# ElementsProject/lightning

Hardware: NVIDIA H100
Metric: secp256k1 verifies/sec (higher is better)
Workload: dtype u32 (8x32-bit limbs, IMAD.WIDE.U32 carry chains)

## Files before the change

### include/cln_sigverify.h

```cpp
#ifndef CLN_SIGVERIFY_H
#define CLN_SIGVERIFY_H

#include <stddef.h>
#include <stdint.h>

#ifdef __cplusplus
extern "C" {
#endif

typedef struct sv_ctx sv_ctx;

#define SV_KIND_ECDSA33 0
#define SV_KIND_ECDSA_XY 1
#define SV_KIND_SCHNORR 2

typedef enum {
    SV_OK = 0,
    SV_ERR_NO_DEVICE = -1,
    SV_ERR_CUDA = -2,
    SV_ERR_NOMEM = -3,
    SV_ERR_ARG = -4
} sv_status;

int sv_create(sv_ctx **out, int device);
// ... 63 lines not shown
int sv_pubkey_parse_host(sv_ctx *ctx, const uint8_t *key33, size_t n, uint8_t *xy64, uint8_t *ok);

enum {
    SV_ST_FE_MUL = 0,
    SV_ST_FE_SQR = 1,
    SV_ST_FE_ADD = 2,
    SV_ST_FE_SUB = 3,
    SV_ST_FE_NEG = 4,
    SV_ST_FE_NORMALIZE = 5,
    SV_ST_FE_INV = 6,
    SV_ST_FE_SQRT = 7,
    SV_ST_FE_MUL3 = 8,
    SV_ST_FE_MUL8 = 9,
    SV_ST_FE_MUL_SMALL = 10,
    SV_ST_FE_DBL = 11,
    SV_ST_FE_B32 = 12,
    SV_ST_U256_MUL_WIDE = 13,
    SV_ST_U256_SQR_WIDE = 14,
    SV_ST_FE_REDUCE512 = 15,
    SV_ST_U256_ADD = 16,
    SV_ST_U256_SUB = 17,
    SV_ST_SC_MUL = 20,
    SV_ST_SC_SQR = 21,
    SV_ST_SC_ADD = 22,
    SV_ST_SC_NEGATE = 23,
    SV_ST_SC_INVERSE = 24,
    SV_ST_SC_REDUCE512 = 25,
    SV_ST_SC_SPLIT_LAMBDA = 26,
    SV_ST_SC_SET_B32 = 27,
    SV_ST_ECMULT_GEN = 28,
    SV_ST_PREPARE_U2 = 29,
    SV_ST_PREPARE_U1 = 30,
    SV_ST_SC_INVERSE_VAR = 31,
    SV_ST_FE_INV_VAR = 32
};
int sv_selftest_host(sv_ctx *ctx, int op, const uint32_t *a, const uint32_t *b, size_t n, uint32_t *out);

int sv_synth_device(sv_ctx *ctx, int kind, uint64_t seed, size_t n, void *d_msg32, void *d_key, void *d_sig64,
                    void *stream);

typedef struct {
    int device;
    int sm_count;
    int main_block;
    int main_grid;
    int main_regs;
    size_t gtable_bytes;
    size_t scratch_bytes;
    unsigned long long launches;
    size_t l2_persist_bytes;
    size_t l2_max_persist_bytes;
} sv_info;
int sv_get_info(const sv_ctx *ctx, sv_info *info);

int sv_set_profiling(sv_ctx *ctx, int on);
int sv_get_last_timing(sv_ctx *ctx, float *prep_ms, float *main_ms);

int sv_probe_imad_peak(sv_ctx *ctx, double *imad_per_sec);
int sv_probe(sv_ctx *ctx, int mode, double *ops_per_sec);

void *sv_host_alloc(size_t bytes);
void sv_host_free(void *p);

#ifdef __cplusplus
}
#endif
#endif
// ... 1 lines not shown
```

### lightning_b200/csrc/engine.cu

```cuda
#include <cuda_runtime.h>
#include <stdio.h>
#include <stdlib.h>
#include <string.h>
#include <string>
#include <vector>

#include "../../include/cln_sigverify.h"
#include "verify.cuh"
#include "selftest.cuh"
#include "batch.cuh"

#if !defined(SV_NO_SYNC_INLINE) && !defined(SV_FE_INLINE)
#error "compile with -DSV_FE_INLINE -DSV_MAIN_SYNC (default build) or -DSV_NO_SYNC_INLINE; see lightning_b200/build.py"
#endif
#ifndef SV_MAIN_BLOCK
#ifdef SV_MAIN_SYNC
#define SV_MAIN_BLOCK 256
#else
#define SV_MAIN_BLOCK 128
#endif
#endif
#ifndef SV_MAIN_MINB
#define SV_MAIN_MINB (512 / SV_MAIN_BLOCK)
#endif
// ... 1676 lines not shown
    memcpy(it.sig, sig64, 64);
    ctx->queue.push_back(it);
    return (long)ctx->queue.size() - 1;
}
extern "C" size_t sv_pending(const sv_ctx* ctx) { return ctx ? ctx->queue.size() : 0; }

extern "C" int sv_flush(sv_ctx* ctx, uint8_t* verdicts, size_t capacity) {
    if (!ctx || (!verdicts && !ctx->queue.empty())) return SV_ERR_ARG;
    size_t total = ctx->queue.size();
    if (capacity < total) return SV_ERR_ARG;
    for (int kind = 0; kind < 3; kind++) {
        size_t ks = sv_key_size(kind);
        std::vector<size_t> idx;
        for (size_t i = 0; i < total; i++)
            if (ctx->queue[i].kind == kind) idx.push_back(i);
        if (idx.empty()) continue;
        size_t m = idx.size();
        std::vector<u8> msg(32 * m), key(ks * m), sig(64 * m), out(m);
        for (size_t j = 0; j < m; j++) {
            const sv_queue_item& it = ctx->queue[idx[j]];
            memcpy(&msg[32 * j], it.msg, 32);
            memcpy(&key[ks * j], it.key, ks);
            memcpy(&sig[64 * j], it.sig, 64);
        }
        int rc = sv_verify_host(ctx, kind, msg.data(), key.data(), sig.data(), m, out.data());
        if (rc) return rc;
        for (size_t j = 0; j < m; j++) verdicts[idx[j]] = out[j];
    }
    ctx->queue.clear();
    return SV_OK;
}

extern "C" int sv_selftest_host(sv_ctx* ctx, int op, const uint32_t* a, const uint32_t* b, size_t n, uint32_t* out) {
    if (!ctx || op < 0 || op > SV_ST_FE_INV_VAR || (n && (!a || !b || !out))) return SV_ERR_ARG;
    if (n == 0) return SV_OK;
    dev_guard dg__;
    CK(dg__.enter(ctx->device));
    dev_tmp ta, tb, to;
    CK(ta.alloc(n * 32));
    CK(tb.alloc(n * 32));
    CK(to.alloc(n * 64));
    cudaStream_t st = ctx->stream;
    CK(cudaMemcpyAsync(ta.p, a, n * 32, cudaMemcpyHostToDevice, st));
    CK(cudaMemcpyAsync(tb.p, b, n * 32, cudaMemcpyHostToDevice, st));
    k_selftest<<<(unsigned)((n + 127) / 128), 128, 0, st>>>(op, ta.as<u32>(), tb.as<u32>(), n, to.as<u32>(), ctx->d_gtab);
    ctx->launches += 1;
    CK(cudaGetLastError());
    CK(cudaMemcpyAsync(out, to.p, n * 64, cudaMemcpyDeviceToHost, st));
    CK(cudaStreamSynchronize(st));
    return SV_OK;
}

extern "C" int sv_synth_device(sv_ctx* ctx, int kind, uint64_t seed, size_t n, void* d_msg32, void* d_key,
                               void* d_sig64, void* stream) {
    if (!ctx || sv_key_size(kind) == 0 || (n && (!d_msg32 || !d_key || !d_sig64))) return SV_ERR_ARG;
    if (n == 0) return SV_OK;
    dev_guard dg__;
    CK(dg__.enter(ctx->device));
    cudaStream_t st = stream ? (cudaStream_t)stream : ctx->stream;
    unsigned grid = (unsigned)((n + 127) / 128);
    if (kind == SV_KIND_ECDSA33)
        k_synth<SV_KIND_ECDSA33><<<grid, 128, 0, st>>>(seed, n, ctx->d_gtab, (u8*)d_msg32, (u8*)d_key, (u8*)d_sig64);
    else if (kind == SV_KIND_ECDSA_XY)
        k_synth<SV_KIND_ECDSA_XY><<<grid, 128, 0, st>>>(seed, n, ctx->d_gtab, (u8*)d_msg32, (u8*)d_key, (u8*)d_sig64);
    else
        k_synth<SV_KIND_SCHNORR><<<grid, 128, 0, st>>>(seed, n, ctx->d_gtab, (u8*)d_msg32, (u8*)d_key, (u8*)d_sig64);
    ctx->launches += 1;
// ... 53 lines not shown
```

### lightning_b200/csrc/fe.cuh

```cuda
#pragma once
#include "u256.cuh"

struct fe {
    u32 v[8];
};

#define SV_P0 0xFFFFFC2Fu
#define SV_P1 0xFFFFFFFEu
#define SV_PC 977u

SV_HD void fe_set_zero(fe& r) {
    SV_UNROLL
    for (int i = 0; i < 8; i++) r.v[i] = 0;
}
SV_HD void fe_set_u32(fe& r, u32 x) {
    fe_set_zero(r);
    r.v[0] = x;
}

SV_HD bool fe_gte_p(const fe& a) {
    u32 hi = a.v[7] & a.v[6] & a.v[5] & a.v[4] & a.v[3] & a.v[2];
    return (hi == 0xFFFFFFFFu) && ((a.v[1] == 0xFFFFFFFFu) || (a.v[1] == SV_P1 && a.v[0] >= SV_P0));
}

// ... 103 lines not shown
            "subc.cc.u32 %5, %5, 0;\n\t"
            "subc.u32 %6, 0, 0;"
            : "+r"(r.v[2]), "+r"(r.v[3]), "+r"(r.v[4]), "+r"(r.v[5]), "+r"(r.v[6]), "+r"(r.v[7]), "=r"(b2));
        b2 &= 1u;
        u32 k2 = b2 * SV_PC;
        asm("sub.cc.u32 %0, %0, %3;\n\t"
            "subc.u32 %1, %1, %2;"
            : "+r"(r.v[0]), "+r"(r.v[1])
            : "r"(b2), "r"(k2));
    }
#else
    u64 d = (u64)r.v[0] - (u64)bw * SV_PC;
    r.v[0] = (u32)d;
    u64 br = (d >> 32) & 1;
    d = (u64)r.v[1] - bw - br;
    r.v[1] = (u32)d;
    br = (d >> 32) & 1;
    for (int i = 2; i < 8; i++) { d = (u64)r.v[i] - br; r.v[i] = (u32)d; br = (d >> 32) & 1; }
    u32 b2 = (u32)br;
    d = (u64)r.v[0] - (u64)b2 * SV_PC;
    r.v[0] = (u32)d;
    br = (d >> 32) & 1;
    r.v[1] = (u32)((u64)r.v[1] - b2 - br);
#endif
}

SV_HD void fe_neg(fe& r, const fe& a) {
    fe z;
    fe_set_zero(z);
    fe_sub(r, z, a);
}
SV_HD void fe_dbl(fe& r, const fe& a) { fe_add(r, a, a); }

SV_HD void fe_reduce512(fe& r, const u32 t[16]) {
#if SV_DEVICE_CODE && defined(SV_REDUCE_SHIFTS)
    u32 s[10];
    s[0] = t[0];
    asm("add.cc.u32 %0, %9, %17;\n\t"
        "addc.cc.u32 %1, %10, %18;\n\t"
        "addc.cc.u32 %2, %11, %19;\n\t"
        "addc.cc.u32 %3, %12, %20;\n\t"
        "addc.cc.u32 %4, %13, %21;\n\t"
        "addc.cc.u32 %5, %14, %22;\n\t"
        "addc.cc.u32 %6, %15, %23;\n\t"
        "addc.cc.u32 %7, %16, 0;\n\t"
        "addc.u32 %8, 0, 0;"
        : "=r"(s[1]), "=r"(s[2]), "=r"(s[3]), "=r"(s[4]), "=r"(s[5]), "=r"(s[6]), "=r"(s[7]), "=r"(s[8]), "=r"(s[9])
        : "r"(t[8]), "r"(t[9]), "r"(t[10]), "r"(t[11]), "r"(t[12]), "r"(t[13]), "r"(t[14]), "r"(t[15]),
          "r"(t[1]), "r"(t[2]), "r"(t[3]), "r"(t[4]), "r"(t[5]), "r"(t[6]), "r"(t[7]));
    u32 h4[9];
    h4[0] = t[8] << 4;
    SV_UNROLL
    for (int k = 1; k < 8; k++) h4[k] = __funnelshift_l(t[8 + k - 1], t[8 + k], 4);
    h4[8] = t[15] >> 28;
    u32 a17[9], a15[9];
    asm("add.cc.u32 %0, %9, %18;\n\t"
        "addc.cc.u32 %1, %10, %19;\n\t"
        "addc.cc.u32 %2, %11, %20;\n\t"
        "addc.cc.u32 %3, %12, %21;\n\t"
        "addc.cc.u32 %4, %13, %22;\n\t"
        "addc.cc.u32 %5, %14, %23;\n\t"
        "addc.cc.u32 %6, %15, %24;\n\t"
        "addc.cc.u32 %7, %16, %25;\n\t"
        "addc.u32 %8, %17, 0;"
        : "=r"(a17[0]), "=r"(a17[1]), "=r"(a17[2]), "=r"(a17[3]), "=r"(a17[4]), "=r"(a17[5]), "=r"(a17[6]), "=r"(a17[7]), "=r"(a17[8])
        : "r"(h4[0]), "r"(h4[1]), "r"(h4[2]), "r"(h4[3]), "r"(h4[4]), "r"(h4[5]), "r"(h4[6]), "r"(h4[7]), "r"(h4[8]),
          "r"(t[8]), "r"(t[9]), "r"(t[10]), "r"(t[11]), "r"(t[12]), "r"(t[13]), "r"(t[14]), "r"(t[15]));
    asm("sub.cc.u32 %0, %9, %18;\n\t"
        "subc.cc.u32 %1, %10, %19;\n\t"
        "subc.cc.u32 %2, %11, %20;\n\t"
        "subc.cc.u32 %3, %12, %21;\n\t"
        "subc.cc.u32 %4, %13, %22;\n\t"
        "subc.cc.u32 %5, %14, %23;\n\t"
        "subc.cc.u32 %6, %15, %24;\n\t"
        "subc.cc.u32 %7, %16, %25;\n\t"
        "subc.u32 %8, %17, 0;"
        : "=r"(a15[0]), "=r"(a15[1]), "=r"(a15[2]), "=r"(a15[3]), "=r"(a15[4]), "=r"(a15[5]), "=r"(a15[6]), "=r"(a15[7]), "=r"(a15[8])
        : "r"(h4[0]), "r"(h4[1]), "r"(h4[2]), "r"(h4[3]), "r"(h4[4]), "r"(h4[5]), "r"(h4[6]), "r"(h4[7]), "r"(h4[8]),
          "r"(t[8]), "r"(t[9]), "r"(t[10]), "r"(t[11]), "r"(t[12]), "r"(t[13]), "r"(t[14]), "r"(t[15]));
    u32 b[9];
    b[0] = a15[0] << 6;
    SV_UNROLL
    for (int k = 1; k < 9; k++) b[k] = __funnelshift_l(a15[k - 1], a15[k], 6);
    asm("add.cc.u32 %0, %0, %10;\n\t"
        "addc.cc.u32 %1, %1, %11;\n\t"
        "addc.cc.u32 %2, %2, %12;\n\t"
        "addc.cc.u32 %3, %3, %13;\n\t"
        "addc.cc.u32 %4, %4, %14;\n\t"
        "addc.cc.u32 %5, %5, %15;\n\t"
        "addc.cc.u32 %6, %6, %16;\n\t"
        "addc.cc.u32 %7, %7, %17;\n\t"
        "addc.cc.u32 %8, %8, %18;\n\t"
        "addc.u32 %9, %9, 0;"
        : "+r"(s[0]), "+r"(s[1]), "+r"(s[2]), "+r"(s[3]), "+r"(s[4]), "+r"(s[5]), "+r"(s[6]), "+r"(s[7]), "+r"(s[8]), "+r"(s[9])
        : "r"(a17[0]), "r"(a17[1]), "r"(a17[2]), "r"(a17[3]), "r"(a17[4]), "r"(a17[5]), "r"(a17[6]), "r"(a17[7]), "r"(a17[8]));
    asm("add.cc.u32 %0, %0, %10;\n\t"
        "addc.cc.u32 %1, %1, %11;\n\t"
        "addc.cc.u32 %2, %2, %12;\n\t"
        "addc.cc.u32 %3, %3, %13;\n\t"
        "addc.cc.u32 %4, %4, %14;\n\t"
        "addc.cc.u32 %5, %5, %15;\n\t"
        "addc.cc.u32 %6, %6, %16;\n\t"
        "addc.cc.u32 %7, %7, %17;\n\t"
        "addc.cc.u32 %8, %8, %18;\n\t"
        "addc.u32 %9, %9, 0;"
        : "+r"(s[0]), "+r"(s[1]), "+r"(s[2]), "+r"(s[3]), "+r"(s[4]), "+r"(s[5]), "+r"(s[6]), "+r"(s[7]), "+r"(s[8]), "+r"(s[9])
        : "r"(b[0]), "r"(b[1]), "r"(b[2]), "r"(b[3]), "r"(b[4]), "r"(b[5]), "r"(b[6]), "r"(b[7]), "r"(b[8]));
    u64 T = ((u64)s[9] << 32) | s[8];
    u64 m = T * SV_PC;
    u64 mid = (m >> 32) + T;
    u32 f0 = (u32)m, f1 = (u32)mid, f2 = (u32)(mid >> 32);
    u32 c;
    asm("add.cc.u32 %0, %9, %17;\n\t"
        "addc.cc.u32 %1, %10, %18;\n\t"
        "addc.cc.u32 %2, %11, %19;\n\t"
        "addc.cc.u32 %3, %12, 0;\n\t"
        "addc.cc.u32 %4, %13, 0;\n\t"
        "addc.cc.u32 %5, %14, 0;\n\t"
        "addc.cc.u32 %6, %15, 0;\n\t"
        "addc.cc.u32 %7, %16, 0;\n\t"
        "addc.u32 %8, 0, 0;"
        : "=r"(r.v[0]), "=r"(r.v[1]), "=r"(r.v[2]), "=r"(r.v[3]), "=r"(r.v[4]), "=r"(r.v[5]), "=r"(r.v[6]),
          "=r"(r.v[7]), "=r"(c)
        : "r"(s[0]), "r"(s[1]), "r"(s[2]), "r"(s[3]), "r"(s[4]), "r"(s[5]), "r"(s[6]), "r"(s[7]), "r"(f0), "r"(f1),
          "r"(f2));
    asm("mad.lo.cc.u32 %0, %3, 977, %0;\n\t"
        "addc.cc.u32 %1, %1, %3;\n\t"
        "addc.u32 %2, %2, 0;"
        : "+r"(r.v[0]), "+r"(r.v[1]), "+r"(r.v[2])
        : "r"(c));
#elif SV_DEVICE_CODE
    u32 s[10];
    s[0] = t[0];
    asm("add.cc.u32 %0, %9, %17;\n\t"
        "addc.cc.u32 %1, %10, %18;\n\t"
        "addc.cc.u32 %2, %11, %19;\n\t"
        "addc.cc.u32 %3, %12, %20;\n\t"
        "addc.cc.u32 %4, %13, %21;\n\t"
        "addc.cc.u32 %5, %14, %22;\n\t"
        "addc.cc.u32 %6, %15, %23;\n\t"
        "addc.cc.u32 %7, %16, 0;\n\t"
        "addc.u32 %8, 0, 0;"
        : "=r"(s[1]), "=r"(s[2]), "=r"(s[3]), "=r"(s[4]), "=r"(s[5]), "=r"(s[6]), "=r"(s[7]), "=r"(s[8]), "=r"(s[9])
        : "r"(t[8]), "r"(t[9]), "r"(t[10]), "r"(t[11]), "r"(t[12]), "r"(t[13]), "r"(t[14]), "r"(t[15]),
          "r"(t[1]), "r"(t[2]), "r"(t[3]), "r"(t[4]), "r"(t[5]), "r"(t[6]), "r"(t[7]));
#ifdef SV_REDUCE_NOACC
    u32 pe[8];
    asm("mul.lo.u32 %0, %8, %12;\n\t"
        "mul.hi.u32 %1, %8, %12;\n\t"
        "mul.lo.u32 %2, %9, %12;\n\t"
        "mul.hi.u32 %3, %9, %12;\n\t"
        "mul.lo.u32 %4, %10, %12;\n\t"
        "mul.hi.u32 %5, %10, %12;\n\t"
        "mul.lo.u32 %6, %11, %12;\n\t"
        "mul.hi.u32 %7, %11, %12;"
        : "=r"(pe[0]), "=r"(pe[1]), "=r"(pe[2]), "=r"(pe[3]), "=r"(pe[4]), "=r"(pe[5]), "=r"(pe[6]), "=r"(pe[7])
        : "r"(t[8]), "r"(t[10]), "r"(t[12]), "r"(t[14]), "r"(SV_PC));
    asm("add.cc.u32 %0, %0, %10;\n\t"
        "addc.cc.u32 %1, %1, %11;\n\t"
        "addc.cc.u32 %2, %2, %12;\n\t"
        "addc.cc.u32 %3, %3, %13;\n\t"
        "addc.cc.u32 %4, %4, %14;\n\t"
        "addc.cc.u32 %5, %5, %15;\n\t"
        "addc.cc.u32 %6, %6, %16;\n\t"
        "addc.cc.u32 %7, %7, %17;\n\t"
        "addc.cc.u32 %8, %8, 0;\n\t"
        "addc.u32 %9, %9, 0;"
        : "+r"(s[0]), "+r"(s[1]), "+r"(s[2]), "+r"(s[3]), "+r"(s[4]), "+r"(s[5]), "+r"(s[6]), "+r"(s[7]),
          "+r"(s[8]), "+r"(s[9])
        : "r"(pe[0]), "r"(pe[1]), "r"(pe[2]), "r"(pe[3]), "r"(pe[4]), "r"(pe[5]), "r"(pe[6]), "r"(pe[7]));
#else
    asm("mad.lo.cc.u32 %0, %10, %14, %0;\n\t"
        "madc.hi.cc.u32 %1, %10, %14, %1;\n\t"
        "madc.lo.cc.u32 %2, %11, %14, %2;\n\t"
        "madc.hi.cc.u32 %3, %11, %14, %3;\n\t"
        "madc.lo.cc.u32 %4, %12, %14, %4;\n\t"
        "madc.hi.cc.u32 %5, %12, %14, %5;\n\t"
        "madc.lo.cc.u32 %6, %13, %14, %6;\n\t"
        "madc.hi.cc.u32 %7, %13, %14, %7;\n\t"
        "addc.cc.u32 %8, %8, 0;\n\t"
        "addc.u32 %9, %9, 0;"
        : "+r"(s[0]), "+r"(s[1]), "+r"(s[2]), "+r"(s[3]), "+r"(s[4]), "+r"(s[5]), "+r"(s[6]), "+r"(s[7]),
          "+r"(s[8]), "+r"(s[9])
        : "r"(t[8]), "r"(t[10]), "r"(t[12]), "r"(t[14]), "r"(SV_PC));
#endif
    u32 o[8];
    asm("mul.lo.u32 %0, %8, %12;\n\t"
        "mul.hi.u32 %1, %8, %12;\n\t"
        "mul.lo.u32 %2, %9, %12;\n\t"
        "mul.hi.u32 %3, %9, %12;\n\t"
        "mul.lo.u32 %4, %10, %12;\n\t"
        "mul.hi.u32 %5, %10, %12;\n\t"
        "mul.lo.u32 %6, %11, %12;\n\t"
        "mul.hi.u32 %7, %11, %12;"
        : "=r"(o[0]), "=r"(o[1]), "=r"(o[2]), "=r"(o[3]), "=r"(o[4]), "=r"(o[5]), "=r"(o[6]), "=r"(o[7])
        : "r"(t[9]), "r"(t[11]), "r"(t[13]), "r"(t[15]), "r"(SV_PC));
    asm("add.cc.u32 %0, %0, %9;\n\t"
        "addc.cc.u32 %1, %1, %10;\n\t"
        "addc.cc.u32 %2, %2, %11;\n\t"
        "addc.cc.u32 %3, %3, %12;\n\t"
        "addc.cc.u32 %4, %4, %13;\n\t"
        "addc.cc.u32 %5, %5, %14;\n\t"
        "addc.cc.u32 %6, %6, %15;\n\t"
        "addc.cc.u32 %7, %7, %16;\n\t"
        "addc.u32 %8, %8, 0;"
        : "+r"(s[1]), "+r"(s[2]), "+r"(s[3]), "+r"(s[4]), "+r"(s[5]), "+r"(s[6]), "+r"(s[7]), "+r"(s[8]), "+r"(s[9])
        : "r"(o[0]), "r"(o[1]), "r"(o[2]), "r"(o[3]), "r"(o[4]), "r"(o[5]), "r"(o[6]), "r"(o[7]));
    u64 T = ((u64)s[9] << 32) | s[8];
    u64 m = T * SV_PC;
    u64 mid = (m >> 32) + T;
    u32 f0 = (u32)m, f1 = (u32)mid, f2 = (u32)(mid >> 32);
    u32 c;
    asm("add.cc.u32 %0, %9, %17;\n\t"
        "addc.cc.u32 %1, %10, %18;\n\t"
        "addc.cc.u32 %2, %11, %19;\n\t"
        "addc.cc.u32 %3, %12, 0;\n\t"
        "addc.cc.u32 %4, %13, 0;\n\t"
        "addc.cc.u32 %5, %14, 0;\n\t"
        "addc.cc.u32 %6, %15, 0;\n\t"
        "addc.cc.u32 %7, %16, 0;\n\t"
        "addc.u32 %8, 0, 0;"
        : "=r"(r.v[0]), "=r"(r.v[1]), "=r"(r.v[2]), "=r"(r.v[3]), "=r"(r.v[4]), "=r"(r.v[5]), "=r"(r.v[6]),
          "=r"(r.v[7]), "=r"(c)
        : "r"(s[0]), "r"(s[1]), "r"(s[2]), "r"(s[3]), "r"(s[4]), "r"(s[5]), "r"(s[6]), "r"(s[7]), "r"(f0), "r"(f1),
          "r"(f2));
    asm("mad.lo.cc.u32 %0, %3, 977, %0;\n\t"
        "addc.cc.u32 %1, %1, %3;\n\t"
        "addc.u32 %2, %2, 0;"
        : "+r"(r.v[0]), "+r"(r.v[1]), "+r"(r.v[2])
        : "r"(c));
#else
    u64 acc = 0;
    u32 s[10];
    for (int i = 0; i < 8; i++) {
        acc += (u64)t[i] + (u64)t[8 + i] * SV_PC;
        if (i > 0) acc += t[8 + i - 1];
        s[i] = (u32)acc;
        acc >>= 32;
    }
    acc += t[15];
    s[8] = (u32)acc;
    s[9] = (u32)(acc >> 32);
    u64 T = ((u64)s[9] << 32) | s[8];
    u64 m = T * SV_PC;
    u64 mid = (m >> 32) + T;
    u32 f[3] = {(u32)m, (u32)mid, (u32)(mid >> 32)};
    u64 c = 0;
    for (int i = 0; i < 8; i++) {
        c += (u64)s[i] + (i < 3 ? f[i] : 0);
        r.v[i] = (u32)c;
        c >>= 32;
    }
    u32 cc = (u32)c;
    u64 q = (u64)r.v[0] + (u64)cc * SV_PC;
    r.v[0] = (u32)q;
    q = (u64)r.v[1] + cc + (q >> 32);
    r.v[1] = (u32)q;
    r.v[2] = (u32)((u64)r.v[2] + (q >> 32));
#endif
}

#if SV_DEVICE_CODE && !defined(SV_FE_INLINE)
static __device__ __noinline__ fe fe_mul_fn(fe a, fe b) {
    u32 t[16];
    fe r;
    u256_mul_wide(t, a.v, b.v);
    fe_reduce512(r, t);
    return r;
}
static __device__ __noinline__ fe fe_sqr_fn(fe a) {
    u32 t[16];
    fe r;
    u256_sqr_wide(t, a.v);
    fe_reduce512(r, t);
    return r;
}
SV_HD void fe_mul(fe& r, const fe& a, const fe& b) { r = fe_mul_fn(a, b); }
SV_HD void fe_sqr(fe& r, const fe& a) { r = fe_sqr_fn(a); }
#else
SV_HD void fe_mul(fe& r, const fe& a, const fe& b) {
    u32 t[16];
    u256_mul_wide(t, a.v, b.v);
    fe_reduce512(r, t);
}
SV_HD void fe_sqr(fe& r, const fe& a) {
    u32 t[16];
    u256_sqr_wide(t, a.v);
    fe_reduce512(r, t);
}
#endif

SV_HD void fe_mul_small(fe& r, const fe& a, u32 k) {
    u64 c = 0;
    u32 s[8];
    SV_UNROLL
    for (int i = 0; i < 8; i++) {
        c += (u64)a.v[i] * k;
        s[i] = (u32)c;
        c >>= 32;
    }
    u64 m = c * SV_PC;
    u64 q = (u64)s[0] + (u32)m;
    r.v[0] = (u32)q;
    q = (u64)s[1] + (m >> 32) + c + (q >> 32);
    r.v[1] = (u32)q;
    SV_UNROLL
    for (int i = 2; i < 8; i++) {
        q = (u64)s[i] + (q >> 32);
        r.v[i] = (u32)q;
    }
    u32 c2 = (u32)(q >> 32);
    q = (u64)r.v[0] + (u64)c2 * SV_PC;
    r.v[0] = (u32)q;
    q = (u64)r.v[1] + c2 + (q >> 32);
    r.v[1] = (u32)q;
    r.v[2] = (u32)((u64)r.v[2] + (q >> 32));
}

SV_HD void fe_mul3(fe& r, const fe& a) {
    fe t;
    fe_add(t, a, a);
    fe_add(r, t, a);
// ... 108 lines not shown
```

### lightning_b200/csrc/ge.cuh

```cuda
#pragma once
#include "fe.cuh"

struct ge {
    fe x, y;
};
struct gej {
    fe x, y, z;
    u32 inf;
};

static SV_CDATA const u32 GE_BETA[8] = {0x719501EEu, 0xC1396C28u, 0x12F58995u, 0x9CF04975u,
                                        0xAC3434E9u, 0x6E64479Eu, 0x657C0710u, 0x7AE96A2Bu};
static SV_CDATA const u32 GE_GX[8] = {0x16F81798u, 0x59F2815Bu, 0x2DCE28D9u, 0x029BFCDBu,
                                      0xCE870B07u, 0x55A06295u, 0xF9DCBBACu, 0x79BE667Eu};
static SV_CDATA const u32 GE_GY[8] = {0xFB10D4B8u, 0x9C47D08Fu, 0xA6855419u, 0xFD17B448u,
                                      0x0E1108A8u, 0x5DA4FBFCu, 0x26A3C465u, 0x483ADA77u};

SV_HD void gej_set_ge(gej& r, const ge& a) {
    r.x = a.x;
    r.y = a.y;
    fe_set_u32(r.z, 1);
    r.inf = 0;
}

SV_HD void gej_double(gej& r, const gej& a) {
    fe A, B, C, D, E, t;
    fe_sqr(A, a.x);
    fe_sqr(B, a.y);
    fe_sqr(C, B);
    fe_add(t, a.x, B);
    fe_sqr(t, t);
    fe_sub(t, t, A);
    fe_sub(t, t, C);
    fe_dbl(D, t);
    fe_mul3(E, A);
    fe_mul(t, a.y, a.z);
    fe_dbl(r.z, t);
    fe_sqr(t, E);
    fe_sub(t, t, D);
    fe_sub(r.x, t, D);
    fe_sub(t, D, r.x);
    fe_mul(t, t, E);
    fe_mul8(C, C);
    fe_sub(r.y, t, C);
    r.inf = a.inf;
}

SV_HD void gej_add_ge(gej& r, const gej& a, const ge& b, fe* rzr = nullptr) {
    if (a.inf) {
        gej_set_ge(r, b);
        if (rzr) fe_set_u32(*rzr, 1);
        return;
    }
    fe zz, u2, s2, h, rr, hh, hhh, v, t;
    fe_sqr(zz, a.z);
    fe_mul(u2, b.x, zz);
    fe_mul(t, a.z, zz);
    fe_mul(s2, b.y, t);
    fe_sub(h, u2, a.x);
    fe_sub(rr, s2, a.y);
    if (fe_is_zero(h)) {
        if (fe_is_zero(rr)) {
            if (rzr) fe_dbl(*rzr, a.y);
            gej_double(r, a);
        } else {
            r.inf = 1;
            if (rzr) fe_set_zero(*rzr);
        }
        return;
    }
    if (rzr) *rzr = h;
    fe_sqr(hh, h);
    fe_mul(hhh, h, hh);
    fe_mul(v, a.x, hh);
    fe_mul(r.z, a.z, h);
    fe_sqr(t, rr);
    fe_sub(t, t, hhh);
    fe_sub(t, t, v);
    fe x3;
    fe_sub(x3, t, v);
    fe_sub(t, v, x3);
    fe_mul(t, t, rr);
    fe_mul(hhh, hhh, a.y);
    fe_sub(r.y, t, hhh);
    r.x = x3;
    r.inf = 0;
}

SV_HD void gej_add_gej(gej& r, const gej& a, const gej& b) {
    if (a.inf) {
        r = b;
        return;
    }
    if (b.inf) {
        r = a;
        return;
    }
    fe z22, z12, u1, u2, s1, s2, h, rr, t;
    fe_sqr(z22, b.z);
    fe_sqr(z12, a.z);
    fe_mul(u1, a.x, z22);
    fe_mul(u2, b.x, z12);
    fe_mul(t, b.z, z22);
    fe_mul(s1, a.y, t);
    fe_mul(t, a.z, z12);
    fe_mul(s2, b.y, t);
    fe_sub(h, u2, u1);
    fe_sub(rr, s2, s1);
    if (fe_is_zero(h)) {
        if (fe_is_zero(rr)) {
            gej_double(r, a);
        } else {
            r.inf = 1;
            fe_set_zero(r.x);
            fe_set_zero(r.y);
            fe_set_zero(r.z);
        }
        return;
// ... 51 lines not shown
```

### lightning_b200/csrc/selftest.cuh

```cuda
#pragma once
#include "../../include/cln_sigverify.h"
#include "verify.cuh"

SV_HD void selftest_item(int op, const u32 A[8], const u32 B[8], u32 R[16], const ge_mem* gtab) {
    SV_UNROLL
    for (int k = 0; k < 16; k++) R[k] = 0;
    fe x, y, r;
    sc p, q, s;
SV_UNROLL
    for (int k = 0; k < 8; k++) { x.v[k] = A[k]; y.v[k] = B[k]; p.v[k] = A[k]; q.v[k] = B[k]; }
    fe_set_zero(r);
    bool is_fe = false, is_sc = false;
    switch (op) {
        case SV_ST_FE_MUL: fe_mul(r, x, y); is_fe = true; break;
        case SV_ST_FE_SQR: fe_sqr(r, x); is_fe = true; break;
        case SV_ST_FE_ADD: fe_add(r, x, y); is_fe = true; break;
        case SV_ST_FE_SUB: fe_sub(r, x, y); is_fe = true; break;
        case SV_ST_FE_NEG: fe_neg(r, x); is_fe = true; break;
        case SV_ST_FE_NORMALIZE: r = x; fe_normalize(r); is_fe = true; R[8] = fe_is_zero(x); R[9] = fe_gte_p(x); R[10] = fe_equal(x, y); break;
        case SV_ST_FE_INV: fe_inv(r, x); is_fe = true; break;
        case SV_ST_FE_SQRT: R[8] = fe_sqrt(r, x) ? 1u : 0u; is_fe = true; break;
        case SV_ST_FE_MUL3: fe_mul3(r, x); is_fe = true; break;
        case SV_ST_FE_MUL8: fe_mul8(r, x); is_fe = true; break;
        case SV_ST_FE_MUL_SMALL: fe_mul_small(r, x, B[0] & 0xFFFFu); is_fe = true; break;
        case SV_ST_FE_DBL: fe_dbl(r, x); is_fe = true; break;
        case SV_ST_FE_B32: {
            u8 bytes[32], back[32];
SV_UNROLL
            for (int k = 0; k < 8; k++) { bytes[4 * k] = (u8)A[k]; bytes[4 * k + 1] = (u8)(A[k] >> 8); bytes[4 * k + 2] = (u8)(A[k] >> 16); bytes[4 * k + 3] = (u8)(A[k] >> 24); }
            R[8] = fe_set_b32(r, bytes) ? 1u : 0u;
            fe_get_b32(back, r);
SV_UNROLL
            for (int k = 0; k < 8; k++) R[k] = (u32)back[4 * k] | ((u32)back[4 * k + 1] << 8) | ((u32)back[4 * k + 2] << 16) | ((u32)back[4 * k + 3] << 24);
            break;
        }
        case SV_ST_U256_MUL_WIDE: u256_mul_wide(R, A, B); break;
        case SV_ST_U256_SQR_WIDE: u256_sqr_wide(R, A); break;
        case SV_ST_FE_REDUCE512: {
            u32 t[16];
SV_UNROLL
            for (int k = 0; k < 8; k++) { t[k] = A[k]; t[8 + k] = B[k]; }
            fe_reduce512(r, t);
            is_fe = true;
            break;
        }
        case SV_ST_U256_ADD: R[8] = u256_add(R, A, B); break;
        case SV_ST_U256_SUB: R[8] = u256_sub(R, A, B); break;
        case SV_ST_SC_MUL: sc_mul(s, p, q); is_sc = true; break;
        case SV_ST_SC_SQR: sc_sqr(s, p); is_sc = true; break;
        case SV_ST_SC_ADD: sc_add(s, p, q); is_sc = true; break;
        case SV_ST_SC_NEGATE: sc_negate(s, p); is_sc = true; R[8] = sc_is_high(p); R[9] = sc_is_zero(p); R[10] = sc_gte_n(A); break;
        case SV_ST_SC_INVERSE: sc_inverse(s, p); is_sc = true; break;
        case SV_ST_SC_INVERSE_VAR: sc_inverse_var(s, p); is_sc = true; break;
        case SV_ST_FE_INV_VAR: fe_inv_var(r, x); is_fe = true; break;
        case SV_ST_SC_REDUCE512: {
            u32 t[16];
SV_UNROLL
            for (int k = 0; k < 8; k++) { t[k] = A[k]; t[8 + k] = B[k]; }
            sc_reduce512(s, t);
            is_sc = true;
            break;
        }
        case SV_ST_SC_SPLIT_LAMBDA: {
            sc r1, r2;
            sc_split_lambda(r1, r2, p);
SV_UNROLL
            for (int k = 0; k < 8; k++) { R[k] = r1.v[k]; R[8 + k] = r2.v[k]; }
            break;
        }
        case SV_ST_SC_SET_B32: {
            u8 bytes[32];
            bool ov;
SV_UNROLL
            for (int k = 0; k < 8; k++) { bytes[4 * k] = (u8)A[k]; bytes[4 * k + 1] = (u8)(A[k] >> 8); bytes[4 * k + 2] = (u8)(A[k] >> 16); bytes[4 * k + 3] = (u8)(A[k] >> 24); }
            sc_set_b32(s, bytes, &ov);
            is_sc = true;
            R[8] = ov ? 1u : 0u;
            break;
        }
        case SV_ST_ECMULT_GEN: {
            ge P;
            if (sc_is_zero(p)) break;
            ecmult_gen_comb(P, p, gtab);
SV_UNROLL
            for (int k = 0; k < 8; k++) { R[k] = P.x.v[k]; R[8 + k] = P.y.v[k]; }
            break;
        }
// ... 26 lines not shown
```

### lightning_b200/csrc/verify.cuh

```cuda
#pragma once
#include "ge.cuh"
#include "sc.cuh"
#include "sha256.cuh"

#define SV_KIND_ECDSA33 0
#define SV_KIND_ECDSA_XY 1
#define SV_KIND_SCHNORR 2
#define SV_KIND_ECDSA33_NS 3
#define SV_KIND_SCHNORR_NS 4

#define SV_GT_ROW 32768
#define SV_GT_ENTRIES (15 * SV_GT_ROW + 65536)

struct alignas(16) ge_mem {
    u32 x[8], y[8];
};
struct alignas(16) qtab_entry {
    u32 x[8], y[8], h[8];
};

SV_HD void ge_from_mem(ge& r, const ge_mem* p) {
#if SV_DEVICE_CODE
    const uint4* q = reinterpret_cast<const uint4*>(p);
    uint4 a = q[0], b = q[1], c = q[2], d = q[3];
// ... 119 lines not shown
        sc_mul(acc, acc, v[i]);
        v[i] = t;
    }
    v[0] = acc;
}


SV_HD bool key_decode(ge& Q, int kind, const u8* key) {
    if (kind == SV_KIND_ECDSA33) {
        u8 pfx = key[0];
        fe x;
        bool ok = (pfx == 2 || pfx == 3);
        ok = fe_set_b32(x, key + 1) && ok;
        return ge_set_xo(Q, x, pfx == 3) && ok;
    } else if (kind == SV_KIND_ECDSA_XY) {
        bool ok = fe_set_b32(Q.x, key);
        ok = fe_set_b32(Q.y, key + 32) && ok;
        return ge_is_on_curve(Q) && ok;
    } else {
        fe x;
        bool ok = fe_set_b32(x, key);
        return ge_set_xo(Q, x, false) && ok;
    }
}

SV_HD u32 window4(const u32* mag, int i) {
    int off = 4 * i + 1;
    int l = off >> 5, sh = off & 31;
    u64 two = ((u64)mag[l + 1] << 32) | mag[l];
    return (u32)(two >> sh) & 15u;
}

SV_HD void qtable_build(qtab_entry* tab, fe& zc, const ge& Q, unsigned sync_threads = 0) {
    gej D, acc;
    gej_set_ge(D, Q);
    gej_double(D, D);
    fe c2, c3;
    fe_sqr(c2, D.z);
    fe_mul(c3, c2, D.z);
    ge d_aff, q1;
    d_aff.x = D.x;
    d_aff.y = D.y;
    fe_mul(q1.x, Q.x, c2);
    fe_mul(q1.y, Q.y, c3);
    gej_set_ge(acc, q1);
    fe_to_words(tab[0].x, q1.x);
    fe_to_words(tab[0].y, q1.y);
#if SV_DEVICE_CODE
#pragma unroll 1
#endif
    for (int k = 1; k < 8; k++) {
        fe h;
        SV_SYNC(sync_threads);
        gej_add_ge(acc, acc, d_aff, &h);
        fe_to_words(tab[k].x, acc.x);
        fe_to_words(tab[k].y, acc.y);
        fe_to_words(tab[k].h, h);
    }
    fe_mul(zc, acc.z, D.z);
    fe zr;
    fe_from_words(zr, tab[7].h);
#if SV_DEVICE_CODE
#pragma unroll 1
#endif
    for (int k = 6; k >= 0; k--) {
        fe zr2, zr3, t;
        fe_sqr(zr2, zr);
        fe_mul(zr3, zr2, zr);
        fe_from_words(t, tab[k].x);
        fe_mul(t, t, zr2);
        fe_to_words(tab[k].x, t);
        fe_from_words(t, tab[k].y);
        fe_mul(t, t, zr3);
        fe_to_words(tab[k].y, t);
        if (k > 0) {
            fe_from_words(t, tab[k].h);
            fe_mul(zr, zr, t);
        }
    }
    fe beta;
    SV_UNROLL
    for (int i = 0; i < 8; i++) beta.v[i] = GE_BETA[i];
#if SV_DEVICE_CODE
#pragma unroll 1
#endif
    for (int k = 0; k < 8; k++) {
        fe t;
        fe_from_words(t, tab[k].x);
        fe_mul(t, t, beta);
        fe_to_words(tab[k].h, t);
    }
}

SV_HD void qtable_fetch(ge& p, const qtab_entry* tab, u32 v, u32 sneg, bool lam) {
    u32 dneg = (v < 8) ? 1u : 0u;
    u32 idx = dneg ? (7u - v) : (v - 8u);
    fe_from_words(p.x, lam ? tab[idx].h : tab[idx].x);
    fe_from_words(p.y, tab[idx].y);
    if (dneg ^ sneg) fe_neg(p.y, p.y);
}

SV_HD void ecmult_ladder_q(gej& R, const sv_work* w, const qtab_entry* tab, const fe& zc, unsigned sync_threads = 0) {
    const u32* m1 = w->k1;
    const u32* m2 = w->k2;
    u32 t1 = m1[4], t2 = m2[4];
    u32 s1 = t1 >> 31, s2 = t2 >> 31;
    ge p;
    {
        u32 v1 = (t1 >> 1) & 7u, v2 = (t2 >> 1) & 7u;
        qtable_fetch(p, tab, v1 + 8u, s1, false);
        gej_set_ge(R, p);
        qtable_fetch(p, tab, v2 + 8u, s2, true);
        gej_add_ge(R, R, p);
    }
#if SV_DEVICE_CODE
#pragma unroll 1
#endif
    for (int i = 31; i >= 0; i--) {
#if SV_DEVICE_CODE
#pragma unroll 1
#endif
#if defined(SV_SYNC_LEVEL) && SV_SYNC_LEVEL < 2
#ifndef SV_SYNC_WINDOWS
#define SV_SYNC_WINDOWS 1
#endif
        if (i % SV_SYNC_WINDOWS == 0) SV_SYNC(sync_threads);
#endif
        for (int j = 0; j < 4; j++) {
#if !defined(SV_SYNC_LEVEL) || SV_SYNC_LEVEL >= 2
            SV_SYNC(sync_threads);
#endif
            gej_double(R, R);
        }
#if SV_DEVICE_CODE
#pragma unroll 1
#endif
        for (int half = 0; half < 2; half++) {
            u32 v = half ? window4(m2, i) : window4(m1, i);
#if !defined(SV_SYNC_LEVEL) || SV_SYNC_LEVEL >= 2
            SV_SYNC(sync_threads);
#endif
            qtable_fetch(p, tab, v, half ? s2 : s1, half != 0);
            gej_add_ge(R, R, p);
        }
    }
    fe_mul(R.z, R.z, zc);
}

SV_HD void ecmult_comb_add(gej& R, const sv_work* w, const ge_mem* gtab, unsigned sync_threads = 0) {
    ge p;
#if defined(SV_COMB_SMEM) && SV_DEVICE_CODE
    {
        extern __shared__ __align__(16) unsigned char sv_smem_raw[];
        const ge_mem* t8 = reinterpret_cast<const ge_mem*>(sv_smem_raw);
        fe beta;
        SV_UNROLL
        for (int i = 0; i < 8; i++) beta.v[i] = GE_BETA[i];
        const u32 top = w->pad[0];
#pragma unroll 1
        for (int row = 0; row < 17; row++) {
            SV_SYNC(sync_threads);
#pragma unroll 1
            for (int half = 0; half < 2; half++) {
                int d;
                if (row < 16) d = half ? (int)(short)((u32)w->gd[row] >> 16) : (int)(short)((u32)w->gd[row] & 0xFFFFu);
                else d = (int)(signed char)((top >> (8 * half)) & 0xFFu);
                u32 sneg = (top >> (16 + half)) & 1u;
                if (d != 0) {
                    u32 a = (u32)(d < 0 ? -d : d);
                    ge_from_mem(p, t8 + (size_t)row * 128 + (a - 1));
                    if (half) fe_mul(p.x, p.x, beta);
                    if ((d < 0) != (sneg != 0)) fe_neg(p.y, p.y);
                    gej_add_ge(R, R, p);
                }
            }
        }
    }
#else
#if SV_DEVICE_CODE
#pragma unroll 1
#endif
    for (int row = 0; row < 16; row++) {
        int d = w->gd[row];
        SV_SYNC(sync_threads);
        if (d != 0) {
            u32 a = (u32)(d < 0 ? -d : d);
            ge_from_mem(p, gtab + (size_t)row * SV_GT_ROW + (a - 1));
            if (d < 0) fe_neg(p.y, p.y);
            gej_add_ge(R, R, p);
        }
    }
#endif
}

SV_HD void ecmult_ladder(gej& R, const sv_work* w, const ge_mem* gtab, const qtab_entry* tab, const fe& zc,
                         unsigned sync_threads = 0) {
    ecmult_ladder_q(R, w, tab, zc, sync_threads);
    ecmult_comb_add(R, w, gtab, sync_threads);
}

SV_HD void ecmult_uniform(gej& R, const sv_work* w, const ge& Q, const ge_mem* gtab, qtab_entry* tab,
                          unsigned sync_threads = 0) {
    fe zc;
    qtable_build(tab, zc, Q, sync_threads);
    ecmult_ladder(R, w, gtab, tab, zc, sync_threads);
}

SV_HD u32 ecdsa_final(const gej& R, const u8* sig64, u32 flags);

struct alignas(16) sv_shared_key {
    qtab_entry tab[8];
    u32 zc[8];
    u32 ok, pad[3];
};
SV_HD void sharedkey_build(sv_shared_key* out, int kind, const u8* key, unsigned sync_threads = 0) {
    ge Q;
    bool ok = key_decode(Q, kind, key);
    fe zc;
    qtable_build(out->tab, zc, Q, sync_threads);
    fe_to_words(out->zc, zc);
    out->ok = ok ? 1u : 0u;
}
// ... 816 lines not shown
```

Before: 44.27 million.

## Fuse mul-add into single reduction and specialize affine point additions

Adds fe_mul_add, which sums two 512-bit products and performs one modular reduction, via a new fe_reduce513 that handles a carry limb. gej_add_ge is rewritten to a doubling-free formula that uses the fused mul-add for the Y coordinate, and a new gej_add_ge_ge handles affine+affine additions with z=h. The Q table build now uses affine-isomorphic doubling and co-Z style additions, and the comb loop uses the cheaper affine+affine add when R is still affine. The goal is to cut the number of field multiplications and reductions per point addition; the cost is extra code paths and carry-handling complexity. The rzr output of gej_add_ge is removed.

```diff
diff --git a/include/cln_sigverify.h b/include/cln_sigverify.h
--- a/include/cln_sigverify.h
+++ b/include/cln_sigverify.h
@@ -119,7 +119,8 @@
     SV_ST_PREPARE_U2 = 29,
     SV_ST_PREPARE_U1 = 30,
     SV_ST_SC_INVERSE_VAR = 31,
-    SV_ST_FE_INV_VAR = 32
+    SV_ST_FE_INV_VAR = 32,
+    SV_ST_FE_MUL_ADD = 33
 };
 int sv_selftest_host(sv_ctx *ctx, int op, const uint32_t *a, const uint32_t *b, size_t n, uint32_t *out);
 
diff --git a/lightning_b200/csrc/engine.cu b/lightning_b200/csrc/engine.cu
--- a/lightning_b200/csrc/engine.cu
+++ b/lightning_b200/csrc/engine.cu
@@ -1732,7 +1732,7 @@
 }
 
 extern "C" int sv_selftest_host(sv_ctx* ctx, int op, const uint32_t* a, const uint32_t* b, size_t n, uint32_t* out) {
-    if (!ctx || op < 0 || op > SV_ST_FE_INV_VAR || (n && (!a || !b || !out))) return SV_ERR_ARG;
+    if (!ctx || op < 0 || op > SV_ST_FE_MUL_ADD || (n && (!a || !b || !out))) return SV_ERR_ARG;
     if (n == 0) return SV_OK;
     dev_guard dg__;
     CK(dg__.enter(ctx->device));
diff --git a/lightning_b200/csrc/fe.cuh b/lightning_b200/csrc/fe.cuh
--- a/lightning_b200/csrc/fe.cuh
+++ b/lightning_b200/csrc/fe.cuh
@@ -159,7 +159,10 @@
 }
 SV_HD void fe_dbl(fe& r, const fe& a) { fe_add(r, a, a); }
 
-SV_HD void fe_reduce512(fe& r, const u32 t[16]) {
+SV_HD void fe_reduce513(fe& r, const u32 t[16], u32 t16) {
+#if SV_DEVICE_CODE
+    const u32 k16 = t16 * SV_PC;
+#endif
 #if SV_DEVICE_CODE && defined(SV_REDUCE_SHIFTS)
     u32 s[10];
     s[0] = t[0];
@@ -171,10 +174,10 @@
         "addc.cc.u32 %5, %14, %22;\n\t"
         "addc.cc.u32 %6, %15, %23;\n\t"
         "addc.cc.u32 %7, %16, 0;\n\t"
-        "addc.u32 %8, 0, 0;"
+        "addc.u32 %8, %24, 0;"
         : "=r"(s[1]), "=r"(s[2]), "=r"(s[3]), "=r"(s[4]), "=r"(s[5]), "=r"(s[6]), "=r"(s[7]), "=r"(s[8]), "=r"(s[9])
         : "r"(t[8]), "r"(t[9]), "r"(t[10]), "r"(t[11]), "r"(t[12]), "r"(t[13]), "r"(t[14]), "r"(t[15]),
-          "r"(t[1]), "r"(t[2]), "r"(t[3]), "r"(t[4]), "r"(t[5]), "r"(t[6]), "r"(t[7]));
+          "r"(t[1]), "r"(t[2]), "r"(t[3]), "r"(t[4]), "r"(t[5]), "r"(t[6]), "r"(t[7]), "r"(t16));
     u32 h4[9];
     h4[0] = t[8] << 4;
     SV_UNROLL
@@ -233,6 +236,10 @@
         "addc.u32 %9, %9, 0;"
         : "+r"(s[0]), "+r"(s[1]), "+r"(s[2]), "+r"(s[3]), "+r"(s[4]), "+r"(s[5]), "+r"(s[6]), "+r"(s[7]), "+r"(s[8]), "+r"(s[9])
         : "r"(b[0]), "r"(b[1]), "r"(b[2]), "r"(b[3]), "r"(b[4]), "r"(b[5]), "r"(b[6]), "r"(b[7]), "r"(b[8]));
+    asm("add.cc.u32 %0, %0, %2;\n\t"
+        "addc.u32 %1, %1, 0;"
+        : "+r"(s[8]), "+r"(s[9])
+        : "r"(k16));
     u64 T = ((u64)s[9] << 32) | s[8];
     u64 m = T * SV_PC;
     u64 mid = (m >> 32) + T;
@@ -267,10 +274,10 @@
         "addc.cc.u32 %5, %14, %22;\n\t"
         "addc.cc.u32 %6, %15, %23;\n\t"
         "addc.cc.u32 %7, %16, 0;\n\t"
-        "addc.u32 %8, 0, 0;"
+        "addc.u32 %8, %24, 0;"
         : "=r"(s[1]), "=r"(s[2]), "=r"(s[3]), "=r"(s[4]), "=r"(s[5]), "=r"(s[6]), "=r"(s[7]), "=r"(s[8]), "=r"(s[9])
         : "r"(t[8]), "r"(t[9]), "r"(t[10]), "r"(t[11]), "r"(t[12]), "r"(t[13]), "r"(t[14]), "r"(t[15]),
-          "r"(t[1]), "r"(t[2]), "r"(t[3]), "r"(t[4]), "r"(t[5]), "r"(t[6]), "r"(t[7]));
+          "r"(t[1]), "r"(t[2]), "r"(t[3]), "r"(t[4]), "r"(t[5]), "r"(t[6]), "r"(t[7]), "r"(t16));
 #ifdef SV_REDUCE_NOACC
     u32 pe[8];
     asm("mul.lo.u32 %0, %8, %12;\n\t"
@@ -291,11 +298,11 @@
         "addc.cc.u32 %5, %5, %15;\n\t"
         "addc.cc.u32 %6, %6, %16;\n\t"
         "addc.cc.u32 %7, %7, %17;\n\t"
-        "addc.cc.u32 %8, %8, 0;\n\t"
+        "addc.cc.u32 %8, %8, %18;\n\t"
         "addc.u32 %9, %9, 0;"
         : "+r"(s[0]), "+r"(s[1]), "+r"(s[2]), "+r"(s[3]), "+r"(s[4]), "+r"(s[5]), "+r"(s[6]), "+r"(s[7]),
           "+r"(s[8]), "+r"(s[9])
-        : "r"(pe[0]), "r"(pe[1]), "r"(pe[2]), "r"(pe[3]), "r"(pe[4]), "r"(pe[5]), "r"(pe[6]), "r"(pe[7]));
+        : "r"(pe[0]), "r"(pe[1]), "r"(pe[2]), "r"(pe[3]), "r"(pe[4]), "r"(pe[5]), "r"(pe[6]), "r"(pe[7]), "r"(k16));
 #else
     asm("mad.lo.cc.u32 %0, %10, %14, %0;\n\t"
         "madc.hi.cc.u32 %1, %10, %14, %1;\n\t"
@@ -305,11 +312,11 @@
         "madc.hi.cc.u32 %5, %12, %14, %5;\n\t"
         "madc.lo.cc.u32 %6, %13, %14, %6;\n\t"
         "madc.hi.cc.u32 %7, %13, %14, %7;\n\t"
-        "addc.cc.u32 %8, %8, 0;\n\t"
+        "addc.cc.u32 %8, %8, %15;\n\t"
         "addc.u32 %9, %9, 0;"
         : "+r"(s[0]), "+r"(s[1]), "+r"(s[2]), "+r"(s[3]), "+r"(s[4]), "+r"(s[5]), "+r"(s[6]), "+r"(s[7]),
           "+r"(s[8]), "+r"(s[9])
-        : "r"(t[8]), "r"(t[10]), "r"(t[12]), "r"(t[14]), "r"(SV_PC));
+        : "r"(t[8]), "r"(t[10]), "r"(t[12]), "r"(t[14]), "r"(SV_PC), "r"(k16));
 #endif
     u32 o[8];
     asm("mul.lo.u32 %0, %8, %12;\n\t"
@@ -365,9 +372,9 @@
         s[i] = (u32)acc;
         acc >>= 32;
     }
-    acc += t[15];
+    acc += (u64)t[15] + (u64)t16 * SV_PC;
     s[8] = (u32)acc;
-    s[9] = (u32)(acc >> 32);
+    s[9] = (u32)(acc >> 32) + t16;
     u64 T = ((u64)s[9] << 32) | s[8];
     u64 m = T * SV_PC;
     u64 mid = (m >> 32) + T;
@@ -386,6 +393,7 @@
     r.v[2] = (u32)((u64)r.v[2] + (q >> 32));
 #endif
 }
+SV_HD void fe_reduce512(fe& r, const u32 t[16]) { fe_reduce513(r, t, 0); }
 
 #if SV_DEVICE_CODE && !defined(SV_FE_INLINE)
 static __device__ __noinline__ fe fe_mul_fn(fe a, fe b) {
@@ -415,6 +423,58 @@
     u256_sqr_wide(t, a.v);
     fe_reduce512(r, t);
 }
+#endif
+
+SV_HD void fe_mul_add_body(fe& r, const fe& a, const fe& b, const fe& c, const fe& d) {
+    u32 t[16], u[16], t16;
+    u256_mul_wide(t, a.v, b.v);
+    u256_mul_wide(u, c.v, d.v);
+#if SV_DEVICE_CODE
+    u32 c8;
+    asm("add.cc.u32 %0, %0, %9;\n\t"
+        "addc.cc.u32 %1, %1, %10;\n\t"
+        "addc.cc.u32 %2, %2, %11;\n\t"
+        "addc.cc.u32 %3, %3, %12;\n\t"
+        "addc.cc.u32 %4, %4, %13;\n\t"
+        "addc.cc.u32 %5, %5, %14;\n\t"
+        "addc.cc.u32 %6, %6, %15;\n\t"
+        "addc.cc.u32 %7, %7, %16;\n\t"
+        "addc.u32 %8, 0, 0;"
+        : "+r"(t[0]), "+r"(t[1]), "+r"(t[2]), "+r"(t[3]), "+r"(t[4]), "+r"(t[5]), "+r"(t[6]), "+r"(t[7]), "=r"(c8)
+        : "r"(u[0]), "r"(u[1]), "r"(u[2]), "r"(u[3]), "r"(u[4]), "r"(u[5]), "r"(u[6]), "r"(u[7]));
+    asm("{\n\t.reg .u32 z;\n\t"
+        "add.cc.u32 z, %17, 0xFFFFFFFF;\n\t"
+        "addc.cc.u32 %0, %0, %9;\n\t"
+        "addc.cc.u32 %1, %1, %10;\n\t"
+        "addc.cc.u32 %2, %2, %11;\n\t"
+        "addc.cc.u32 %3, %3, %12;\n\t"
+        "addc.cc.u32 %4, %4, %13;\n\t"
+        "addc.cc.u32 %5, %5, %14;\n\t"
+        "addc.cc.u32 %6, %6, %15;\n\t"
+        "addc.cc.u32 %7, %7, %16;\n\t"
+        "addc.u32 %8, 0, 0;\n\t}"
+        : "+r"(t[8]), "+r"(t[9]), "+r"(t[10]), "+r"(t[11]), "+r"(t[12]), "+r"(t[13]), "+r"(t[14]), "+r"(t[15]), "=r"(t16)
+        : "r"(u[8]), "r"(u[9]), "r"(u[10]), "r"(u[11]), "r"(u[12]), "r"(u[13]), "r"(u[14]), "r"(u[15]), "r"(c8));
+#else
+    u64 acc = 0;
+    for (int i = 0; i < 16; i++) {
+        acc += (u64)t[i] + u[i];
+        t[i] = (u32)acc;
+        acc >>= 32;
+    }
+    t16 = (u32)acc;
+#endif
+    fe_reduce513(r, t, t16);
+}
+#if SV_DEVICE_CODE && !defined(SV_FE_INLINE)
+static __device__ __noinline__ fe fe_mul_add_fn(fe a, fe b, fe c, fe d) {
+    fe r;
+    fe_mul_add_body(r, a, b, c, d);
+    return r;
+}
+SV_HD void fe_mul_add(fe& r, const fe& a, const fe& b, const fe& c, const fe& d) { r = fe_mul_add_fn(a, b, c, d); }
+#else
+SV_HD void fe_mul_add(fe& r, const fe& a, const fe& b, const fe& c, const fe& d) { fe_mul_add_body(r, a, b, c, d); }
 #endif
 
 SV_HD void fe_mul_small(fe& r, const fe& a, u32 k) {
diff --git a/lightning_b200/csrc/ge.cuh b/lightning_b200/csrc/ge.cuh
--- a/lightning_b200/csrc/ge.cuh
+++ b/lightning_b200/csrc/ge.cuh
@@ -46,13 +46,12 @@
     r.inf = a.inf;
 }
 
-SV_HD void gej_add_ge(gej& r, const gej& a, const ge& b, fe* rzr = nullptr) {
+SV_HD void gej_add_ge(gej& r, const gej& a, const ge& b) {
     if (a.inf) {
         gej_set_ge(r, b);
-        if (rzr) fe_set_u32(*rzr, 1);
         return;
     }
-    fe zz, u2, s2, h, rr, hh, hhh, v, t;
+    fe zz, u2, s2, h, rr, hh, i, j, v, t;
     fe_sqr(zz, a.z);
     fe_mul(u2, b.x, zz);
     fe_mul(t, a.z, zz);
@@ -61,29 +60,60 @@
     fe_sub(rr, s2, a.y);
     if (fe_is_zero(h)) {
         if (fe_is_zero(rr)) {
-            if (rzr) fe_dbl(*rzr, a.y);
             gej_double(r, a);
         } else {
             r.inf = 1;
-            if (rzr) fe_set_zero(*rzr);
         }
         return;
     }
-    if (rzr) *rzr = h;
+    fe_dbl(rr, rr);
+    fe_sqr(hh, h);
+    fe_dbl(i, hh);
+    fe_dbl(i, i);
+    fe_mul(j, h, i);
+    fe_mul(v, a.x, i);
+    fe_add(t, a.z, h);
+    fe_sqr(t, t);
+    fe_sub(t, t, zz);
+    fe_sub(r.z, t, hh);
+    fe x3;
+    fe_sqr(x3, rr);
+    fe_sub(x3, x3, j);
+    fe_sub(x3, x3, v);
+    fe_sub(x3, x3, v);
+    fe_sub(v, v, x3);
+    fe_dbl(j, j);
+    fe_neg(t, a.y);
+    fe_mul_add(r.y, rr, v, j, t);
+    r.x = x3;
+    r.inf = 0;
+}
+
+SV_HD void gej_add_ge_ge(gej& r, const ge& a, const ge& b) {
+    fe h, rr, hh, hhh, v, t, x3;
+    fe_sub(h, b.x, a.x);
+    fe_sub(rr, b.y, a.y);
+    if (fe_is_zero(h)) {
+        gej_set_ge(r, a);
+        if (fe_is_zero(rr)) {
+            gej_double(r, r);
+        } else {
+            r.inf = 1;
+        }
+        return;
+    }
     fe_sqr(hh, h);
     fe_mul(hhh, h, hh);
     fe_mul(v, a.x, hh);
-    fe_mul(r.z, a.z, h);
-    fe_sqr(t, rr);
-    fe_sub(t, t, hhh);
-    fe_sub(t, t, v);
-    fe x3;
-    fe_sub(x3, t, v);
-    fe_sub(t, v, x3);
-    fe_mul(t, t, rr);
-    fe_mul(hhh, hhh, a.y);
-    fe_sub(r.y, t, hhh);
+    fe_sqr(x3, rr);
+    fe_sub(x3, x3, hhh);
+    fe_sub(x3, x3, v);
+    fe_sub(x3, x3, v);
+    fe_sub(v, v, x3);
+    fe_neg(t, a.y);
+    fe_mul_add(r.y, rr, v, hhh, t);
     r.x = x3;
+    r.z = h;
     r.inf = 0;
 }
 
diff --git a/lightning_b200/csrc/selftest.cuh b/lightning_b200/csrc/selftest.cuh
--- a/lightning_b200/csrc/selftest.cuh
+++ b/lightning_b200/csrc/selftest.cuh
@@ -53,6 +53,7 @@
         case SV_ST_SC_INVERSE: sc_inverse(s, p); is_sc = true; break;
         case SV_ST_SC_INVERSE_VAR: sc_inverse_var(s, p); is_sc = true; break;
         case SV_ST_FE_INV_VAR: fe_inv_var(r, x); is_fe = true; break;
+        case SV_ST_FE_MUL_ADD: fe_mul_add(r, x, x, y, y); is_fe = true; break;
         case SV_ST_SC_REDUCE512: {
             u32 t[16];
 SV_UNROLL
diff --git a/lightning_b200/csrc/verify.cuh b/lightning_b200/csrc/verify.cuh
--- a/lightning_b200/csrc/verify.cuh
+++ b/lightning_b200/csrc/verify.cuh
@@ -175,32 +175,54 @@
 }
 
 SV_HD void qtable_build(qtab_entry* tab, fe& zc, const ge& Q, unsigned sync_threads = 0) {
-    gej D, acc;
-    gej_set_ge(D, Q);
-    gej_double(D, D);
-    fe c2, c3;
-    fe_sqr(c2, D.z);
-    fe_mul(c3, c2, D.z);
-    ge d_aff, q1;
-    d_aff.x = D.x;
-    d_aff.y = D.y;
-    fe_mul(q1.x, Q.x, c2);
-    fe_mul(q1.y, Q.y, c3);
-    gej_set_ge(acc, q1);
-    fe_to_words(tab[0].x, q1.x);
-    fe_to_words(tab[0].y, q1.y);
+    ge d, acc;
+    {
+        fe A, B, C, E, t;
+        fe_sqr(A, Q.x);
+        fe_sqr(B, Q.y);
+        fe_sqr(C, B);
+        fe_add(t, Q.x, B);
+        fe_sqr(t, t);
+        fe_sub(t, t, A);
+        fe_sub(t, t, C);
+        fe_dbl(acc.x, t);
+        fe_mul8(acc.y, C);
+        fe_mul3(E, A);
+        fe_sqr(t, E);
+        fe_sub(t, t, acc.x);
+        fe_sub(d.x, t, acc.x);
+        fe_sub(t, acc.x, d.x);
+        fe_mul(t, t, E);
+        fe_sub(d.y, t, acc.y);
+        fe_dbl(t, Q.y);
+        fe_to_words(tab[0].h, t);
+    }
+    fe_to_words(tab[0].x, acc.x);
+    fe_to_words(tab[0].y, acc.y);
 #if SV_DEVICE_CODE
 #pragma unroll 1
 #endif
     for (int k = 1; k < 8; k++) {
-        fe h;
+        fe h, c, w1, w2, rr, t;
         SV_SYNC(sync_threads);
-        gej_add_ge(acc, acc, d_aff, &h);
+        fe_sub(h, acc.x, d.x);
+        fe_sqr(c, h);
+        fe_mul(w1, d.x, c);
+        fe_mul(w2, acc.x, c);
+        fe_sub(rr, acc.y, d.y);
+        fe_sub(t, w2, w1);
+        fe_mul(d.y, d.y, t);
+        d.x = w1;
+        fe_sqr(t, rr);
+        fe_sub(t, t, w1);
+        fe_sub(acc.x, t, w2);
+        fe_sub(t, w1, acc.x);
+        fe_mul(t, t, rr);
+        fe_sub(acc.y, t, d.y);
         fe_to_words(tab[k].x, acc.x);
         fe_to_words(tab[k].y, acc.y);
         fe_to_words(tab[k].h, h);
     }
-    fe_mul(zc, acc.z, D.z);
     fe zr;
     fe_from_words(zr, tab[7].h);
 #if SV_DEVICE_CODE
@@ -221,6 +243,11 @@
             fe_mul(zr, zr, t);
         }
     }
+    {
+        fe z2;
+        fe_from_words(z2, tab[0].h);
+        fe_mul(zc, zr, z2);
+    }
     fe beta;
     SV_UNROLL
     for (int i = 0; i < 8; i++) beta.v[i] = GE_BETA[i];
@@ -251,10 +278,10 @@
     ge p;
     {
         u32 v1 = (t1 >> 1) & 7u, v2 = (t2 >> 1) & 7u;
-        qtable_fetch(p, tab, v1 + 8u, s1, false);
-        gej_set_ge(R, p);
+        ge p1;
+        qtable_fetch(p1, tab, v1 + 8u, s1, false);
         qtable_fetch(p, tab, v2 + 8u, s2, true);
-        gej_add_ge(R, R, p);
+        gej_add_ge_ge(R, p1, p);
     }
 #if SV_DEVICE_CODE
 #pragma unroll 1
@@ -320,6 +347,7 @@
         }
     }
 #else
+    u32 affine = 0;
 #if SV_DEVICE_CODE
 #pragma unroll 1
 #endif
@@ -330,7 +358,18 @@
             u32 a = (u32)(d < 0 ? -d : d);
             ge_from_mem(p, gtab + (size_t)row * SV_GT_ROW + (a - 1));
             if (d < 0) fe_neg(p.y, p.y);
-            gej_add_ge(R, R, p);
+            if (R.inf) {
+                gej_set_ge(R, p);
+                affine = 1;
+            } else if (affine) {
+                ge q;
+                q.x = R.x;
+                q.y = R.y;
+                gej_add_ge_ge(R, q, p);
+                affine = 0;
+            } else {
+                gej_add_ge(R, R, p);
+            }
         }
     }
 #endif
```

Measured after the change: 44.77 million, median of 6. 1.1% higher.
